# northflank-examples/distributed-pytorch-example

Measured on AMD Instinct MI355X. Metric: samples/sec (whole node) + DDP scaling eff., ResNet-50 bf16 at 1/2/4/8 MI355X, higher is better.
Workload: dtype bf16; 1 GPU; model=resnet50-v1.5, global_batch=512, per_gpu_batch=512, grad_accum=1, parallelism=dp1, optimizer=sgd-momentum0.9

## Files before the change

### csrc/bindings/bn.cpp

```cpp
#include <algorithm>
#include <vector>

#include "../kernels/pwconv.h"
#include "gemm_plan.h"
#include "ops_common.h"

namespace dpe_ops {
namespace {

int64_t rows_of(const Tensor& x) { return x.numel() / x.size(-1); }

std::vector<Tensor> bn_fwd_train(const Tensor& x, const c10::optional<Tensor>& gamma, const c10::optional<Tensor>& beta,
                                 const c10::optional<Tensor>& rmean, const c10::optional<Tensor>& rvar, double momentum,
                                 double eps, bool relu, const c10::optional<Tensor>& residual,
                                 const c10::optional<Tensor>& stats) {
  CHECK_GPU(x); CHECK_BF16(x); CHECK_CONTIG(x);
  const int64_t C = x.size(-1), M = rows_of(x);
  TORCH_CHECK(C % 8 == 0 && C <= 2048, "bn: C must be a multiple of 8 and <= 2048");
  auto fo = x.options().dtype(at::kFloat);
  Tensor coef = at::empty({4, C}, fo);
  hipStream_t st = cur_stream();
  if (has(stats)) {
    TORCH_CHECK(stats->dim() == 3 && stats->size(0) == 2 && stats->size(1) == C, "stats must be [2][C][nb] partials");
    CHECK_RC(dpe_bn_finalize(fp(*stats), (int)stats->size(2), (int)C, M, fpo(gamma), fpo(beta), fpom(rmean), fpom(rvar),
// ... 182 lines not shown
  const int64_t M = xshape[0] * xshape[1] * xshape[2], C = xshape[3];
  return (C == 64 || C == 128) && cmid == C && dpe_pw_cat_fwd_rowgroups(M, cout, C) > 0;
}

std::vector<Tensor> conv1x1_apply_cat(const Tensor& x, const Tensor& w, const c10::optional<Tensor>& in_coef,
                                      const Tensor& out_coef, const Tensor& x2, const Tensor& w2, const Tensor& coef2) {
  CHECK_GPU(x); CHECK_BF16(x); CHECK_CONTIG(x); CHECK_BF16(w); CHECK_CONTIG(w); CHECK_F32(out_coef); CHECK_CONTIG(out_coef);
  CHECK_GPU(x2); CHECK_BF16(x2); CHECK_CONTIG(x2); CHECK_BF16(w2); CHECK_CONTIG(w2); CHECK_F32(coef2); CHECK_CONTIG(coef2);
  const int64_t K1 = x.size(-1), M = x.numel() / K1, N = w.size(0), K2 = x2.size(-1);
  TORCH_CHECK(x.dim() == 4 && K1 == K2 && x2.numel() == M * K2 && w.numel() == N * K1 && w2.numel() == N * K2 &&
                  out_coef.numel() == 4 * N && coef2.numel() == 4 * N, "conv1x1_apply_cat: shapes");
  if (has(in_coef)) {
    CHECK_F32((*in_coef)); CHECK_CONTIG((*in_coef));
    TORCH_CHECK(in_coef->numel() == 4 * K1, "conv1x1_apply_cat: in_coef must be the BN's [4][K] coefficients");
  }
  TORCH_CHECK(down_cat_ok(x2.sizes().vec(), K1, N, 1), "conv1x1_apply_cat: outside the envelope (down_cat_ok)");
  const int rg = dpe_pw_cat_fwd_rowgroups(M, N, K2);
  auto ysz = x.sizes().vec();
  ysz.back() = N;
  Tensor y = at::empty(ysz, x.options());
  auto bsz = ysz;
  bsz.back() = N / 8;
  Tensor bits = at::empty(bsz, x.options().dtype(at::kByte));
  dpe::PwArgs pa{};
  pa.x = bp(x); pa.w = bp(w); pa.y = bpm(y);
  pa.x2 = bp(x2); pa.w2 = bp(w2); pa.cat_k2 = (int)K2;
  pa.in_coef = fpo(in_coef);
  pa.out_coef = fp(out_coef);
  pa.res_coef = fp(coef2);
  pa.out_bits = (uint8_t*)bits.data_ptr();
  pa.M = M; pa.N = N; pa.K = K1 + K2; pa.rg = rg; pa.sched = dpe_gemm::sched_buffer(cur_stream());
  CHECK_RC(dpe_pw_launch(&pa, dpe::PW_CAT, cur_stream()), "pw_stream concatenated-K apply");
  return {y, bits};
}

std::vector<Tensor> bn_gram_bwd(const Tensor& part, const Tensor& P, const Tensor& w, const Tensor& u, const Tensor& sv,
                                const Tensor& coef, const c10::optional<Tensor>& gamma, int64_t M,
                                const c10::optional<Tensor>& dgamma, const c10::optional<Tensor>& dbeta, Tensor& dw) {
  CHECK_GPU(part); CHECK_F32(part); CHECK_F32(P); CHECK_F32(u); CHECK_F32(sv); CHECK_F32(coef); CHECK_F32(dw);
  CHECK_BF16(w); CHECK_CONTIG(w); CHECK_CONTIG(P); CHECK_CONTIG(dw); CHECK_CONTIG(part);
  const int64_t Cout = w.size(0), Cin = w.numel() / Cout;
  TORCH_CHECK(part.dim() == 3 && part.size(1) == Cout && P.numel() == Cout * Cin && u.numel() == Cout * Cin &&
                  dw.numel() == Cout * Cin && sv.numel() == 2 * Cin && coef.numel() == 4 * Cout && sv.is_contiguous(),
              "bn_gram_bwd: shapes");
  auto fo = P.options();
  Tensor bcat = at::empty({Cout + Cin, Cin}, w.options()), abc = at::empty({3, Cout}, fo), e = at::empty({Cin}, fo);
  Tensor qws = at::empty({dpe_gram_bwd_ws_floats((int)Cin, (int)Cout)}, fo);
  CHECK_RC(dpe_gram_bwd(fp(part), (int)part.size(2), fp(P), bp(w), fp(u), fp(sv), fp(coef), fpo(gamma), (int)Cin,
                        (int)Cout, M, fpom(dgamma), fpom(dbeta), fp(dw), bpm(bcat), fp(abc), fp(e), fp(qws), cur_stream()),
           "bn_gram_bwd");
  return {bcat, e};
}

std::vector<Tensor> conv1x1_dgrad_cat(const Tensor& dz, const Tensor& a2src, const c10::optional<Tensor>& a2_coef,
                                      const Tensor& bcat, const Tensor& e, const Tensor& bn_x, const Tensor& bn_coef) {
  CHECK_GPU(dz); CHECK_BF16(dz); CHECK_CONTIG(dz); CHECK_BF16(a2src); CHECK_CONTIG(a2src); CHECK_BF16(bcat);
  CHECK_CONTIG(bcat); CHECK_F32(e); CHECK_BF16(bn_x); CHECK_CONTIG(bn_x); CHECK_F32(bn_coef);
  const int64_t K1 = dz.size(-1), M = dz.numel() / K1, C = a2src.size(-1);
  TORCH_CHECK(a2src.numel() == M * C && bcat.size(0) == K1 + C && bcat.size(1) == C && e.numel() == C &&
                  bn_x.sizes() == a2src.sizes() && bn_coef.numel() == 4 * C && K1 % 32 == 0 && C % 32 == 0,
              "conv1x1_dgrad_cat: shapes");
  Tensor dx = at::empty_like(bn_x);
  if (hgemm_conv_on() && !has(a2_coef) && C >= 256 && C % 64 == 0 && K1 % 64 == 0) {
    int pcols = 0;
    const auto pl = dpe_gemm::plan_bnb(M, C, K1 + C, 1, 0, &pcols);
    if (pl.cfg >= 0 && pl.splits == 1 && pcols > 0) {
// ... 364 lines not shown

}

void register_bn(pybind11::module& m) {
  namespace py = pybind11;
  m.def("gram_ok", [](std::vector<int64_t> h2shape, int64_t cout3, int64_t next_width) {
          if (h2shape.size() != 4 || !pw_stream_on()) return false;
          const int64_t M = h2shape[0] * h2shape[1] * h2shape[2], C2 = h2shape[3];
          if (C2 != 64 && C2 != 128 && C2 != 256) return false;
          if (cout3 % 128 || M % 32) return false;
          return dpe_pw_rowgroups(M, cout3, C2, dpe::PW_APPLY) > 0 &&
                 dpe_pw_rowgroups(M, cout3, next_width, dpe::PW_DSUM) > 0;
        }, py::arg("h2_shape"), py::arg("cout3"), py::arg("next_width"));
  m.def("bn_gram", &bn_gram, py::arg("x"), py::arg("coef") = py::none(), py::arg("shift_coef") = py::none(),
        py::arg("stride2") = false,
        "(G = a'^T a', s = [colsum(a'), mu]) of a' = a2 - mu, a2 = relu(x * coef[0] + coef[1]) (or x), centred on the "
        "pilot shift of shift_coef (default coef); fp32, deterministic");
  m.def("bn_gram_coef", &bn_gram_coef, py::arg("G"), py::arg("s"), py::arg("w"), py::arg("M"), py::arg("gamma"),
        py::arg("beta"), py::arg("running_mean"), py::arg("running_var"), py::arg("momentum"), py::arg("eps"),
        "BN coefficients [4][Cout] of the never-computed h = a2 W^T from (G, s), and u = W G");
  m.def("conv1x1_apply", &conv1x1_apply, py::arg("x"), py::arg("w"), py::arg("in_coef"), py::arg("out_coef"),
        py::arg("residual"), py::arg("res_coef") = py::none(),
        "y = relu(BN(x' W^T) + residual [BN_d]) and its ReLU bits (pre-BN tensor never stored)");
  m.def("conv1x1_apply_next", &conv1x1_apply_next, py::arg("x"), py::arg("w"), py::arg("in_coef"), py::arg("out_coef"),
        py::arg("residual"), py::arg("res_coef"), py::arg("w_next"), py::arg("outs") = py::none(),
        "conv1x1_apply's (y, bits) and, from the same pass, the next conv1's h1 = y W_next^T with its BN-forward partials");
  m.def("c1_fuse_ok", &c1_fuse_ok, py::arg("h2_shape"), py::arg("cout3"), py::arg("c1_next"),
        "conv1x1_apply_next's envelope: conv3 64 -> 256 beside a 1x1 stride-1 conv1 256 -> {64, 128}; no CU budget");
  m.def("conv1x1_apply_cat", &conv1x1_apply_cat, py::arg("x"), py::arg("w"), py::arg("in_coef"), py::arg("out_coef"),
        py::arg("x2"), py::arg("w2"), py::arg("coef2"),
        "y = relu(BN3(x' W^T) + BN_d(x2 W2^T)) over the concatenated K and its ReLU bits (no pre-BN tensors)");
  m.def("down_cat_ok", &down_cat_ok, py::arg("xshape"), py::arg("cmid"), py::arg("cout"), py::arg("stride"),
        "conv1x1_apply_cat's envelope: 1x1 stride-1 downsample conv, Cin == cmid in {64, 128}, cout == 4 Cin");
  m.def("bn_gram_bwd", &bn_gram_bwd, py::arg("part"), py::arg("P"), py::arg("w"), py::arg("u"), py::arg("s"),
        py::arg("coef"), py::arg("gamma"), py::arg("M"), py::arg("dgamma"), py::arg("dbeta"), py::arg("dw"),
        "BN3 backward from (sum dz partials, P = dz^T a2): dgamma/dbeta/dw +=, returns (B_cat bf16, bias)");
  m.def("conv1x1_dgrad_cat", &conv1x1_dgrad_cat, py::arg("dz"), py::arg("a2src"), py::arg("a2_coef"), py::arg("bcat"),
        py::arg("e"), py::arg("bn_x"), py::arg("bn_coef"),
        "[dz | a2] x bcat + e with the BN2-backward partials (concatenated-K data grad)");
  m.def("bn_gram_pilot", &bn_gram_pilot, py::arg("x"), py::arg("stride2") = false,
        "pilot shift [4][C] for bn_gram's shift_coef from a sample of x's rows (x without a producing BN)");
  m.def("bn_gram_u", &bn_gram_u, py::arg("G"), py::arg("w"), "u = W G (fp32) alone: no coefficients, no running stats");
  m.def("conv1x1_dgrad_cat_plain", &conv1x1_dgrad_cat_plain, py::arg("dz"), py::arg("x"), py::arg("bcat"), py::arg("e"),
        py::arg("stride2") = false,
        "[dz | x] x bcat + e (concatenated-K data grad of a Gram-path downsample branch, no partials)");
  m.def("bnd_gram_ok", [](std::vector<int64_t> xshape, int64_t cout, std::vector<int64_t> stride) {
          if (xshape.size() != 4 || stride.size() != 2 || stride[0] != stride[1] || !igemm_dma_on()) return false;
          const int64_t M = xshape[0] * xshape[1] * xshape[2], C = xshape[3];
          if (stride[0] == 1) return (C == 64 || C == 128) && cout == 4 * C && dpe_pw_cat_blocks(M, cout, C) > 0;
          if (stride[0] != 2 || xshape[1] % 2 || xshape[2] % 2) return false;
          static const bool gdma = env_on("DPE_GRAM_DMA", true);
          const int64_t Mo = M / 4, lim = (1ll << 31) - 4096;
          return gdma && (C == 64 || C == 128 || C == 256) && cout >= 256 && cout % 32 == 0 && hgemm_conv_on() &&
                 hgemm_conv_wgrad_on() && Mo % 64 == 0 && Mo < (1 << 24) && M * C * 2 < lim && Mo * cout * 2 < lim;
        }, py::arg("xshape"), py::arg("cout"), py::arg("stride"));
  m.def("bn_bwd_coef", &bn_bwd_coef, py::arg("partials"), py::arg("M"), py::arg("gamma"), py::arg("coef"),
        py::arg("dgamma") = py::none(), py::arg("dbeta") = py::none(),
        "BN-backward coefficients [3][C] from the dgrad-epilogue partials (no apply pass); dgamma/dbeta +=");
  m.def("conv1x1_bnin_fwd", &conv1x1_bnin_fwd, py::arg("h"), py::arg("res"), py::arg("coef"), py::arg("res_coef"),
        py::arg("w"), py::arg("x_out"), py::arg("x_bits"), py::arg("want_stats") = true, py::arg("tile_m") = 128,
        "1x1 conv over x = relu(BN(h) + res [BN_d]) computed on load; x (+ ReLU bits) stored as a by-product");
  m.def("conv1x1_bnin_dgrad", &conv1x1_bnin_dgrad, py::arg("dz"), py::arg("h"), py::arg("bcoef"), py::arg("w"),
        py::arg("dh_out"), py::arg("bn_x"), py::arg("bn_coef"),
        "1x1 data grad over dh = a*dz + b*h + c computed on load (dh stored as a by-product) + BN-backward partials");
  m.def("bn_coef", &bn_coef, py::arg("stats"), py::arg("M"), py::arg("gamma"), py::arg("beta"), py::arg("running_mean"),
        py::arg("running_var"), py::arg("momentum"), py::arg("eps"));
// ... 30 lines not shown
```

### csrc/kernels/pwconv.h

```cpp
#pragma once
#include <hip/hip_runtime.h>
#include <stdint.h>

namespace dpe {

enum PwEpi : int {
  PW_FWD = 0,
  PW_DGRAD = 1,
  PW_APPLY = 2,
  PW_DSUM = 3,
  PW_CAT = 4,
};

struct PwArgs {
  const uint16_t* x;
  const uint16_t* w;
  uint16_t* y;
  float* stats;
  const uint16_t* residual;
  const uint8_t* res_mask;
  const uint16_t* st_x;
  const float* st_coef;
  const uint8_t* st_mask;
  int64_t M, N, K;
// ... 11 lines not shown
  const uint16_t* x2;
  const uint16_t* w2;
  int cat_k2;
  const uint16_t* w_next;
  uint16_t* y_next;
  float* stats_next;
  int c1_next;
};

struct PwCatArgs {
  const uint16_t* dz;
  const uint16_t* h2;
  const float* coef;
  const uint16_t* bcat;
  const float* ebias;
  uint16_t* y;
  float* stats;
  int64_t M;
  int rg;
};

}

extern "C" int dpe_pw_cat_blocks(int64_t M, int64_t K1, int64_t K2);
extern "C" int dpe_pw_cat_launch(const dpe::PwCatArgs* args, int64_t K1, int64_t K2, hipStream_t stream);

extern "C" int dpe_pw_rowgroups(int64_t M, int64_t N, int64_t K, int epi);
extern "C" int dpe_pw_launch(const dpe::PwArgs* args, int epi, hipStream_t stream);

extern "C" int dpe_pw_cat_fwd_rowgroups(int64_t M, int64_t N, int64_t k2);

extern "C" int dpe_pw_p_rowgroups(int64_t M, int64_t N, int64_t K, int64_t k2);
extern "C" int dpe_pw_next_rowgroups(int64_t M, int64_t N, int64_t K, int64_t c1);

extern "C" int dpe_pw_p_reduce(const float* slab, int rg, int64_t n, float* P, hipStream_t stream);
```

### csrc/kernels/pwconv.hip

```cpp
#include <algorithm>
#include <cstdlib>

#include "common.h"
#include "igemm.h"
#include "launch.h"
#include "pwconv.h"

namespace dpe {
namespace pw {

constexpr int BM = 64;
typedef __attribute__((address_space(3))) void lds_void_t;

DPE_DEVICE int kimg_off(int row, int chunk) {
  const int g = (0x78 >> (((row >> 2) & 3) << 1)) & 3;
  return row * 64 + ((chunk ^ g) << 4);
}
DPE_DEVICE bf16x8 kfrag(const char* img, int r0) {
  const int lane = threadIdx.x & 63;
  return __builtin_bit_cast(bf16x8, *(const u32x4*)(img + kimg_off(r0 + (lane & 15), lane >> 4)));
}
DPE_DEVICE __amdgpu_buffer_rsrc_t rsrc(const void* base, uint32_t bytes) {
  return __builtin_amdgcn_make_buffer_rsrc(const_cast<void*>(base), (short)0, (int)bytes, 0x00020000);
}
template <int N>
DPE_DEVICE void wait_vm() {
  static_assert(N >= 0 && N < 64, "vmcnt");
  asm volatile("" ::: "memory");
  __builtin_amdgcn_s_waitcnt((N & 15) | (7 << 4) | (15 << 8) | ((N >> 4) << 14));
  asm volatile("" ::: "memory");
}

template <int C>
DPE_DEVICE int p_h(int row) {
  return C >= 128 ? ((row & 3) | (((row >> 3) & 1) << 2)) : (((row >> 1) & 1) | (((row >> 3) & 1) << 1));
}
typedef __attribute__((address_space(3))) s16x4 lds_s16x4_t;
DPE_DEVICE bf16x8 p_trfrag(const char* a1, const char* a2) {
  const s16x4 lo = __builtin_amdgcn_ds_read_tr16_b64_v4i16((lds_s16x4_t*)a1);
  const s16x4 hi = __builtin_amdgcn_ds_read_tr16_b64_v4i16((lds_s16x4_t*)a2);
  s16x8 r;
  r[0] = lo[0]; r[1] = lo[1]; r[2] = lo[2]; r[3] = lo[3];
  r[4] = hi[0]; r[5] = hi[1]; r[6] = hi[2]; r[7] = hi[3];
  return __builtin_bit_cast(bf16x8, r);
}

template <int K, int WN, int NS, int EPI, bool DYN = false, int K2 = 0, int C1 = 0>
__global__ __launch_bounds__(256, (K == 64 && (EPI == PW_FWD || (K2 > 0 && !DYN))) ? 3 : 2) void pw_stream_kernel(PwArgs a) {
  constexpr int KC = K / 32;
  constexpr int TILE = BM * K * 2;
  constexpr int P = TILE / 1024 / 4;
  constexpr int NI = WN / 16, MI = BM / 16;
  static_assert(P >= 1 && P * 4096 == TILE, "pieces");
  constexpr int ROWB = WN * 2 + 16, CPRW = WN / 8, RPP = 64 / CPRW, NPS = 32 / RPP;
  constexpr int STG = 32 * ROWB;
  constexpr bool NX = C1 > 0;
  static_assert(!NX || (EPI == PW_APPLY && K == 64 && WN == 64 && K2 == 0 && !DYN && (C1 == 64 || C1 == 128)), "next conv1: envelope");
  constexpr int HP = NX ? C1 / 64 : 0;
  constexpr int S = (EPI == PW_APPLY || EPI == PW_CAT ? 4 : 2) * NPS + 2 * HP;
  constexpr int VM = (NX && (NS - 1) * S + (NS - 2) * P > 63) ? 63 : (NS - 1) * S + (NS - 2) * P;
  static_assert(VM < 64, "vmcnt range");
  constexpr bool CAT = EPI == PW_CAT;
  static_assert(!CAT || (WN == 32 && 2 * K2 == K && K2 % 64 == 0), "concatenated K: envelope");
  constexpr int KS = CAT ? K2 : K;
  constexpr int KC1 = KS / 32;
  constexpr bool PF = K2 > 0 && !CAT;
  static_assert(!PF || (EPI == PW_DSUM && WN == 32 && (K2 == 64 || K2 == 128) && K2 <= K), "fused P: envelope");
  constexpr int A2OFF = NS * TILE + 4 * STG + 2 * K * 4 + 16, A2RB = 2 * (PF ? K2 : 8);
  constexpr int H1RB = C1 * 2 + 16, HCPR = NX ? C1 / 8 : 8, HRPP = 64 / HCPR;
  __shared__ __attribute__((aligned(16))) char smem[A2OFF + (PF ? BM * A2RB : NX ? 32 * H1RB : 0)];
  float* const bnin = (float*)(smem + NS * TILE + 4 * STG);
  int* const claim_slot = (int*)(smem + NS * TILE + 4 * STG + 2 * K * 4);

  constexpr bool DG = EPI == PW_DGRAD || EPI == PW_DSUM;
  const int tid = threadIdx.x, lane = tid & 63, g = lane >> 4, li = lane & 15;
  const int wid = __builtin_amdgcn_readfirstlane(tid >> 6);
  const int M = (int)a.M, N = (int)a.N, RG = a.rg;
  const int nbN = N / (4 * WN);
  const int bid = xcd_remap(blockIdx.x, gridDim.x);
  const int nb = bid % nbN;
  int rg = bid / nbN;
  const int SRG = (int)gridDim.x / nbN;
  const int n0w = nb * 4 * WN + wid * WN;
  const int tiles = (M + BM - 1) / BM;
  const int ch = lane % CPRW;
  const int nch = n0w + ch * 8;

  bf16x8 wf[NI][KC];
#pragma unroll
  for (int ni = 0; ni < NI; ++ni)
#pragma unroll
    for (int kc = 0; kc < KC; ++kc) {
      const int n = n0w + 16 * ni + li, k0 = 32 * kc + 8 * g;
      if constexpr (CAT) {
        const uint16_t* const ws = kc < KC1 ? a.w : a.w2;
        wf[ni][kc] = __builtin_bit_cast(bf16x8, *(const u32x4*)(ws + (int64_t)n * KS + (k0 - (kc < KC1 ? 0 : KS))));
      } else if constexpr (!DG) {
        wf[ni][kc] = __builtin_bit_cast(bf16x8, *(const u32x4*)(a.w + (int64_t)n * K + k0));
      } else {
        s16x8 v;
#pragma unroll
        for (int e = 0; e < 8; ++e) v[e] = (short)a.w[(int64_t)(k0 + e) * N + n];
        wf[ni][kc] = __builtin_bit_cast(bf16x8, v);
// ... 58 lines not shown
#pragma unroll
      for (int nj = 0; nj < PNJ; ++nj) pacc[ni][nj] = f32x4{0.f, 0.f, 0.f, 0.f};
  }
  float osc[8], osh[8], rsc[8], rsh[8];
  if constexpr (EPI == PW_APPLY) {
#pragma unroll
    for (int e = 0; e < 8; ++e) {
      osc[e] = a.out_coef[nch + e];
      osh[e] = a.out_coef[N + nch + e];
      rsc[e] = (!NX && a.res_coef) ? a.res_coef[nch + e] : 1.f;
      rsh[e] = (!NX && a.res_coef) ? a.res_coef[N + nch + e] : 0.f;
    }
  }
  const int rh = a.res_h, rw = a.res_w;
  auto res_off = [&](int m) -> int64_t {
    if (rh <= 0) return (int64_t)m * N + nch;
    const int hw = rh * rw, n = m / hw, r = m - n * hw, h = r / rw, w = r - h * rw;
    if ((h | w) & 1) return -1;
    return ((int64_t)(n * (rh >> 1) + (h >> 1)) * (rw >> 1) + (w >> 1)) * N + nch;
  };

  constexpr uint32_t OOB = 0xfffffff0u;
  const uint32_t ybytes = (uint32_t)((int64_t)M * N * 2), mbytes = (uint32_t)((int64_t)M * N / 8);
  const uint32_t rbytes = rh > 0 ? (uint32_t)((int64_t)(M / (rh * rw)) * (rh >> 1) * (rw >> 1) * N * 2) : ybytes;
  const __amdgpu_buffer_rsrc_t yrs = rsrc(a.y, ybytes);
  const __amdgpu_buffer_rsrc_t rrs = rsrc(a.residual, a.residual ? rbytes : 0u);
  const __amdgpu_buffer_rsrc_t rmrs = rsrc(a.res_mask, a.res_mask ? mbytes : 0u);
  const __amdgpu_buffer_rsrc_t xsrs = rsrc(a.st_x, bnx ? ybytes : 0u);
  const __amdgpu_buffer_rsrc_t smrs = rsrc(a.st_mask, (bnb && a.st_mask) ? mbytes : 0u);
  const __amdgpu_buffer_rsrc_t obrs = rsrc(a.out_bits, ((EPI == PW_APPLY || CAT) && a.out_bits) ? mbytes : 0u);
  const __amdgpu_buffer_rsrc_t psrs = rsrc(a.p_src, PF ? (uint32_t)((int64_t)M * K2 * 2) : 0u);
  const __amdgpu_buffer_rsrc_t h1rs = rsrc(a.y_next, NX ? (uint32_t)((int64_t)M * C1 * 2) : 0u);

  if (!DG && a.in_coef) {
    for (int i = tid; i < 2 * KS; i += 256) bnin[i] = a.in_coef[i];
    __syncthreads();
  }
  float c1s[CAT ? NI : 1][4], c2s[CAT ? NI : 1][4], cbs[CAT ? NI : 1][4];
  if constexpr (CAT) {
#pragma unroll
    for (int ni = 0; ni < NI; ++ni)
#pragma unroll
      for (int e = 0; e < 4; ++e) {
        const int n = n0w + 16 * ni + 4 * g + e;
        c1s[ni][e] = a.out_coef[n];
        c2s[ni][e] = a.res_coef[n];
        cbs[ni][e] = a.out_coef[N + n] + a.res_coef[N + n];
      }
  }
  if constexpr (PF) {
    if (a.p_coef)
      for (int i = tid; i < 2 * K2; i += 256) bnin[i] = a.p_coef[i];
    __syncthreads();
  }

  auto tile_body = [&](const int m0, const int cur_slot, const int nxt_tile, const int nxt_slot) {
    constexpr bool HOIST = (EPI != PW_FWD) && (WN == 32 || NX);
    constexpr bool HLD = HOIST && !CAT;
    constexpr int HN = HLD ? NPS : 1;
    u32x4 hrv[2][HN], hxv[2][HN];
    uint32_t hrmb[2][HN], hsmb[2][HN];
    if constexpr (HLD) {
#pragma unroll
      for (int hf = 0; hf < 2; ++hf)
#pragma unroll
        for (int ps = 0; ps < HN; ++ps) {
          const int m = min(m0 + 32 * hf + ps * RPP + lane / CPRW, M - 1);
          const int64_t off = (int64_t)m * N + nch;
          const int64_t ro = EPI == PW_APPLY ? off : res_off(m);
          if (a.residual) hrv[hf][ps] = __builtin_amdgcn_raw_buffer_load_b128(rrs, ro >= 0 ? (uint32_t)(ro * 2) : OOB, 0, 0);
          if constexpr (DG) {
            if (a.res_mask) hrmb[hf][ps] = __builtin_amdgcn_raw_buffer_load_b8(rmrs, (uint32_t)(off >> 3), 0, 0);
// ... 69 lines not shown
      wait_vm<P>();
      char* const a2 = smem + A2OFF;
      if (a.p_coef) {
        int ol = lane;
        asm volatile("" : "+v"(ol));
#pragma unroll
        for (int k = 0; k < PPW; ++k) {
          const int q = wid * PPW + k, r = q * PRPP + ol / PCPR, lc = (ol % PCPR) ^ (2 * p_h<K2>(r));
          const f32x4 s0 = *(const f32x4*)(bnin + 8 * lc), s1 = *(const f32x4*)(bnin + 8 * lc + 4);
          const f32x4 h0 = *(const f32x4*)(bnin + K2 + 8 * lc), h1 = *(const f32x4*)(bnin + K2 + 8 * lc + 4);
          const float sc8[8] = {s0[0], s0[1], s0[2], s0[3], s1[0], s1[1], s1[2], s1[3]};
          const float sh8[8] = {h0[0], h0[1], h0[2], h0[3], h1[0], h1[1], h1[2], h1[3]};
          u32x4* const pc = (u32x4*)(a2 + q * 1024 + ol * 16);
          float f[8];
          unpack8(*pc, f);
#pragma unroll
          for (int e = 0; e < 8; ++e) f[e] = fmaxf(fmaf(f[e], sc8[e], sh8[e]), 0.f);
          *pc = pack8(f);
        }
      }
    }
    char* stg = smem + NS * TILE + wid * STG;
#pragma unroll
    for (int hf = 0; hf < 2; ++hf) {
      if constexpr (NX) {
#pragma unroll
        for (int kc = 0; kc < KC; ++kc) {
          bf16x8 xf[2];
#pragma unroll
          for (int mh = 0; mh < 2; ++mh) xf[mh] = kfrag(img + kc * (BM * 64), 16 * (2 * hf + mh));
#pragma unroll
          for (int mh = 0; mh < 2; ++mh)
#pragma unroll
            for (int ni = 0; ni < NI; ++ni)
              acc[2 * hf + mh][ni] = __builtin_amdgcn_mfma_f32_16x16x32_bf16(wf[ni][kc], xf[mh], acc[2 * hf + mh][ni], 0, 0, 0);
        }
      }
      u32x4 rv[NPS], xv[NPS];
      uint32_t rmb[NPS], smb[NPS];
      if constexpr (HLD) {
#pragma unroll
        for (int ps = 0; ps < HN; ++ps) {
          rv[ps] = hrv[hf][ps];
          xv[ps] = hxv[hf][ps];
          rmb[ps] = a.res_mask ? hrmb[hf][ps] : 0xffu;
          smb[ps] = (bnb && a.st_mask) ? hsmb[hf][ps] : 0xffu;
        }
      } else if constexpr (DG) {
#pragma unroll
        for (int ps = 0; ps < NPS; ++ps) {
          const int m = min(m0 + 32 * hf + ps * RPP + lane / CPRW, M - 1);
          const int64_t off = (int64_t)m * N + nch;
          if (a.residual) {
            const int64_t ro = res_off(m);
            rv[ps] = ro >= 0 ? *(const u32x4*)(a.residual + ro) : u32x4{0u, 0u, 0u, 0u};
          }
          rmb[ps] = a.res_mask ? (uint32_t)a.res_mask[off >> 3] : 0xffu;
          if (bnx) xv[ps] = *(const u32x4*)(a.st_x + off);
          smb[ps] = (bnb && a.st_mask) ? (uint32_t)a.st_mask[off >> 3] : 0xffu;
        }
      }
#pragma unroll
      for (int mh = 0; mh < 2; ++mh) {
        const int mi = 2 * hf + mh;
#pragma unroll
        for (int ni = 0; ni < NI; ++ni) {
          if constexpr (CAT) {
#pragma unroll
            for (int e = 0; e < 4; ++e)
              acc[mi][ni][e] = fmaxf(fmaf(acc[mi][ni][e], c1s[ni][e], fmaf(acc2[mi][ni][e], c2s[ni][e], cbs[ni][e])), 0.f);
          }
          u32x2 pk;
          pk[0] = pack_bf2(acc[mi][ni][0], acc[mi][ni][1]);
          pk[1] = pack_bf2(acc[mi][ni][2], acc[mi][ni][3]);
          *(u32x2*)(stg + (16 * mh + li) * ROWB + (16 * ni + 4 * g) * 2) = pk;
        }
      }
      if (HLD && hf == 0) wait_vm<P>();
#pragma unroll
      for (int ps = 0; ps < NPS; ++ps) {
        const int row = ps * RPP + lane / CPRW;
        u32x4 v = *(const u32x4*)(stg + row * ROWB + ch * 16);
        const int m = m0 + 32 * hf + row;
        const bool valid = m < M;
        float f[8];
        unpack8(v, f);
        if constexpr (EPI == PW_APPLY) {
          float r[8];
          if (a.residual) unpack8(rv[ps], r);
#pragma unroll
          for (int e = 0; e < 8; ++e) {
            float t = fmaf(f[e], osc[e], osh[e]);
            if (a.residual) t += (!NX && a.res_coef) ? bf2f(f2bf(fmaf(r[e], rsc[e], rsh[e]))) : r[e];
            f[e] = fmaxf(t, 0.f);
          }
          v = pack8(f);
          if constexpr (HOIST)
            __builtin_amdgcn_raw_buffer_store_b8(relu_mask_byte(v), obrs, valid ? (uint32_t)(((int64_t)m * N + nch) >> 3) : OOB, 0, 0);
          else if (valid && a.out_bits)
            a.out_bits[((int64_t)m * N + nch) >> 3] = relu_mask_byte(v);
// ... 523 lines not shown
  }
  if (K != 64 && K != 128 && K != 256) return {0, 0};
  if (epi != PW_FWD && epi != PW_DGRAD && epi != PW_APPLY && epi != PW_DSUM && epi != PW_CAT) return {0, 0};
  const int bnb = 4 * pw_wn((int)K, epi);
  if (N % bnb || N < 2 * K) return {0, 0};
  if (M * K * 2 >= (1ll << 31) - 4096 || M * N >= (1ll << 31) - 256) return {0, 0};
  const int64_t tiles = (M + pw::BM - 1) / pw::BM;
  const int64_t nbN = N / bnb;
  const int reserve = dpe_cu_reserve();
  if (reserve > 0 && pw_dynamic()) {
    if (k2 == 128 && epi != PW_CAT) return {0, 0};
    const int64_t srg = std::max<int64_t>(1, (pw_cap<true>(K, epi, k2) - reserve) / nbN);
    static const int64_t fac = [] { const char* e = getenv("DPE_PW_DYN_FACTOR"); return (int64_t)(e ? std::max(2, atoi(e)) : 8); }();
    const int64_t rg = std::min<int64_t>(fac * srg, tiles / 7);
    if (rg > srg) return {(int)rg, (int)srg};
  }
  int64_t rg = (pw_cap<false>(K, epi, k2) - reserve) / nbN;
  rg = std::max<int64_t>(1, std::min<int64_t>(rg, tiles));
  return {(int)rg, (int)rg};
}

static int pw_plan_next(int64_t M, int64_t N, int64_t K, int64_t c1) {
  if (K != 64 || N != 256 || (c1 != 64 && c1 != 128)) return 0;
  if (M <= 0 || M * N >= (1ll << 31) - 256) return 0;
  const int reserve = dpe_cu_reserve();
  if (reserve > 0 && pw_dynamic()) return 0;
  const int cap = c1 == 64 ? pw_slots<64, 64, 4, PW_APPLY, false, 0, 64>() : pw_slots<64, 64, 4, PW_APPLY, false, 0, 128>();
  const int64_t tiles = (M + pw::BM - 1) / pw::BM;
  return (int)std::max<int64_t>(1, std::min<int64_t>(cap - reserve, tiles));
}

extern "C" int dpe_pw_next_rowgroups(int64_t M, int64_t N, int64_t K, int64_t c1) { return pw_plan_next(M, N, K, c1); }

extern "C" int dpe_pw_rowgroups(int64_t M, int64_t N, int64_t K, int epi) { return pw_plan(M, N, K, epi).rg; }

extern "C" int dpe_pw_cat_fwd_rowgroups(int64_t M, int64_t N, int64_t k2) {
  return (k2 > 0 && N == 4 * k2) ? pw_plan(M, N, 2 * k2, PW_CAT, k2).rg : 0;
}

extern "C" int dpe_pw_p_rowgroups(int64_t M, int64_t N, int64_t K, int64_t k2) {
  return k2 > 0 ? pw_plan(M, N, K, PW_DSUM, k2).rg : 0;
}

__global__ __launch_bounds__(256) void pw_p_reduce_kernel(const float* __restrict__ slab, int rg, int64_t n,
                                                          float* __restrict__ P) {
  __shared__ float part[8][32];
  const int o = threadIdx.x & 31, q = threadIdx.x >> 5;
  const int64_t i = (int64_t)blockIdx.x * 32 + o;
  float t = 0.f;
  if (i < n) {
    int r = q;
    for (; r + 56 < rg; r += 64) {
      float v[8];
#pragma unroll
      for (int k = 0; k < 8; ++k) v[k] = slab[(int64_t)(r + 8 * k) * n + i];
#pragma unroll
      for (int k = 0; k < 8; ++k) t += v[k];
    }
    for (; r < rg; r += 8) t += slab[(int64_t)r * n + i];
  }
  part[q][o] = t;
  __syncthreads();
  if (q == 0 && i < n) {
    float u = 0.f;
#pragma unroll
    for (int k = 0; k < 8; ++k) u += part[k][o];
    P[i] = u;
  }
}

extern "C" int dpe_pw_p_reduce(const float* slab, int rg, int64_t n, float* P, hipStream_t st) {
  if (rg <= 0 || n <= 0) return -1;
  hipLaunchKernelGGL(pw_p_reduce_kernel, dim3((unsigned)((n + 31) / 32)), dim3(256), 0, st, slab, rg, n, P);
  return 0;
}

extern "C" int dpe_pw_launch(const PwArgs* args, int epi, hipStream_t st) {
  const PwArgs& a = *args;
  if (a.p_k2 < 0 || (a.p_k2 > 0 && (epi != PW_DSUM || !a.p_src || !a.p_slab))) return -1;
  if ((epi == PW_CAT) != (a.cat_k2 > 0) || (epi == PW_CAT && a.p_k2 > 0)) return -1;
  if (a.c1_next != 0) {
    if (epi != PW_APPLY || a.p_k2 != 0 || !a.w_next || !a.y_next || !a.stats_next || !a.out_coef || !a.residual || a.res_coef ||
        !a.out_bits || a.st_x || a.stats || a.res_h > 0)
      return -1;
    if (a.rg <= 0 || a.rg != pw_plan_next(a.M, a.N, a.K, a.c1_next)) return -1;
    const dim3 grid((unsigned)a.rg), block(256);
    if (a.c1_next == 64) hipLaunchKernelGGL((pw::pw_stream_kernel<64, 64, 4, PW_APPLY, false, 0, 64>), grid, block, 0, st, a);
    else hipLaunchKernelGGL((pw::pw_stream_kernel<64, 64, 4, PW_APPLY, false, 0, 128>), grid, block, 0, st, a);
    return 0;
  }
  const int64_t k2 = epi == PW_CAT ? a.cat_k2 : a.p_k2;
  if (a.rg <= 0 || a.rg != pw_plan(a.M, a.N, a.K, epi, k2).rg) return -1;
  if (epi == PW_CAT && (!a.x2 || !a.w2 || !a.out_coef || !a.res_coef || !a.out_bits || a.residual || a.st_x || a.stats ||
                        a.res_h > 0))
    return -1;
  if (epi == PW_FWD && (a.residual || a.st_x)) return -1;
  if (a.st_x && !a.st_coef) return -1;
  if (epi == PW_DSUM && (a.st_x || !a.st_mask || !a.stats)) return -1;
  if (epi == PW_APPLY && (!a.out_coef || a.st_x || a.stats || a.res_h > 0 || (a.res_coef && !a.residual))) return -1;
  if (a.res_h > 0 && ((epi != PW_DGRAD && epi != PW_DSUM) || a.res_mask || a.res_h % 2 || a.res_w % 2 || a.M % ((int64_t)a.res_h * a.res_w)))
    return -1;
  const int srg = a.sched ? pw_plan(a.M, a.N, a.K, epi, k2).srg : a.rg;
  const bool dyn = srg < a.rg;
  const int wn = pw_wn((int)a.K, epi);
  const dim3 grid((unsigned)(srg * (a.N / (4 * wn)))), block(256);
#define PW_GO(K_, WN_, NS_, E_)                                                                            \
  if (a.K == K_ && wn == WN_ && epi == E_) {                                                             \
    if (dyn) hipLaunchKernelGGL((pw::pw_stream_kernel<K_, WN_, NS_, E_, true>), grid, block, 0, st, a);    \
    else hipLaunchKernelGGL((pw::pw_stream_kernel<K_, WN_, NS_, E_, false>), grid, block, 0, st, a);       \
    return 0;                                                                                            \
  }
#define PW_GO_P(K_, NS_, K2_)                                                                                \
  if (a.K == K_ && a.p_k2 == K2_) {                                                                        \
// ... 32 lines not shown
```

### distributed_pytorch_example_amd/models/_resnet_fused.py

```python
from __future__ import annotations

import os

import torch
from torch.autograd import Function

from ..ops._ext import ext
from ..ops._state import finalize_stream, grad_done, grad_sink, note_use, run_on_aux, shadow

_EPI_BNB = os.environ.get("DPE_BN_EPI", "1") != "0"
_BN3_CHAIN = _EPI_BNB and os.environ.get("DPE_BN3_CHAIN", "1") != "0"
_BN_DUAL = os.environ.get("DPE_BN_DUAL", "1") != "0"
_ROW_BNIN = _EPI_BNB and os.environ.get("DPE_ROW_BNIN", "1") != "0"
_PW_BNIN = _EPI_BNB and os.environ.get("DPE_PW_BNIN", "1") != "0"
_DOWN_CHAIN = _BN3_CHAIN and os.environ.get("DPE_DOWN_CHAIN", "1") != "0"
_AX_FWD = _BN3_CHAIN and os.environ.get("DPE_AX_FWD", "0") == "1"
_AX_BWD = _BN3_CHAIN and os.environ.get("DPE_AX_BWD", "0") == "1"
_AX_BWD_MAXC = int(os.environ.get("DPE_AX_BWD_MAXC", "512"))
_AX_TILE = int(os.environ.get("DPE_AX_TILE", "256"))
_GRAM = _BN3_CHAIN and os.environ.get("DPE_BN3_GRAM", "1") != "0"
_BND_GRAM = _GRAM and os.environ.get("DPE_BND_GRAM", "1") != "0"
_BND_GRAM_S2 = _BND_GRAM and os.environ.get("DPE_BND_GRAM_S2", "0") == "1"
_PW_FUSED_P = _GRAM and os.environ.get("DPE_PW_FUSED_P", "1") != "0"
_DOWN_CAT =_BND_GRAM and os.environ.get("DPE_DOWN_CAT", "1") != "0"
_C1_FUSE = _GRAM and os.environ.get("DPE_C1_FUSE", "1") != "0"


def _ax_ok(conv, cin) -> bool:
    return (tuple(conv.kernel_size) == (1, 1) and tuple(conv.stride) == (1, 1) and tuple(conv.padding) == (0, 0)
            and cin % 32 == 0 and cin <= 2048)


def can_materialise_input(block) -> bool:
    return _AX_FWD and block.fused and _ax_ok(block.c1.conv, block.c1.conv.in_channels)


def _out_hw(hw, conv):
    k, s, p, d = conv.kernel_size[0], conv.stride[0], conv.padding[0], conv.dilation[0]
    return (hw + 2 * p - d * (k - 1) - 1) // s + 1


class _BN3Link:

    __slots__ = ("h3", "coef", "mask", "part", "dz_ptr", "dz_shape", "pending", "gram", "psrc", "P", "h1_next")

    def __init__(self):
        self.h3 = self.coef = self.mask = self.part = None
        self.psrc = self.P = None
        self.dz_ptr, self.dz_shape = 0, None
        self.gram = False
        self.pending = None
        self.h1_next = None


def _conv_conf(conv):
    return list(conv.stride), list(conv.padding), list(conv.dilation)


# ... 34 lines not shown
        def conv_coef(i, inp, in_coef=None):
            cb = convs[i]
            s, p, d = _conv_conf(cb.conv)
            if i == 0 and h1_done is not None:
                h, st = h1_done
            else:
                h, st = C.conv_fwd(inp, ws[i], s, p, d, True, None, in_coef)
            bn = cb.bn
            M = h.numel() // h.shape[-1]
            return h, C.bn_coef(st, M, bn.weight.detach(), bn.bias.detach(), bn.running_mean, bn.running_var, bn.momentum,
                                bn.eps)

        c1conv, c2conv = convs[0].conv, convs[1].conv
        h1_shape = [x.shape[0], _out_hw(x.shape[1], c1conv), _out_hw(x.shape[2], c1conv), c1conv.out_channels]
        h2_shape = [x.shape[0], _out_hw(h1_shape[1], c2conv), _out_hw(h1_shape[2], c2conv), c2conv.out_channels]
        out_shape = [*h2_shape[:3], convs[2].conv.out_channels]
        dconv = block.down.conv if block.down is not None else None
        use_gram = bool(gram_next and link_out is not None and not defer_out and h1_st is None
                        and (gram_next > 0 or C.pw_dgrad_strided_residual_ok(out_shape, -gram_next))
                        and C.gram_ok(h2_shape, convs[2].conv.out_channels, abs(gram_next)))
        bnd_gram = bool(use_gram and _BND_GRAM and dconv is not None and tuple(dconv.kernel_size) == (1, 1)
                        and tuple(dconv.padding) == (0, 0)
                        and C.bnd_gram_ok(list(x.shape), dconv.out_channels, list(dconv.stride))
                        and (tuple(dconv.stride) == (1, 1) or (_BND_GRAM_S2 and tuple(c1conv.stride) == (1, 1) and
                             C.pw_dgrad_strided_residual_ok(list(x.shape), c1conv.out_channels))))
        down_cat = bool(use_gram and _DOWN_CAT and dconv is not None and tuple(dconv.kernel_size) == (1, 1)
                        and tuple(dconv.padding) == (0, 0) and tuple(dconv.stride) == (1, 1)
                        and C.down_cat_ok(list(x.shape), h2_shape[3], dconv.out_channels, 1))
        c1n = next_block.c1.conv if next_block is not None else None
        c1_fuse = bool(use_gram and _C1_FUSE and c1n is not None and block.down is None and gram_next
                       and tuple(c1n.kernel_size) == (1, 1) and tuple(c1n.stride) == (1, 1)
                       and tuple(c1n.padding) == (0, 0) and c1n.in_channels == out_shape[3] and c1n.out_channels == abs(gram_next)
                       and C.c1_fuse_ok(h2_shape, out_shape[3], c1n.out_channels))
        if h1_st is None and block.down is not None and not down_cat:
            hd, cd = conv_coef(3, x)
        else:
            hd, cd = None, None
        if _ROW_BNIN and C.row_bn_on_load(h1_shape, list(ws[1].shape), *_conv_conf(c2conv)):
            h1, c1 = conv_coef(0, x)
            a1 = None
            h2, st2 = C.conv_fwd(h1, ws[1], *_conv_conf(c2conv), True, None, c1)
        else:
            h1, a1, c1 = convbn(0, x, True)
            h2, st2 = C.conv_fwd(a1, ws[1], *_conv_conf(c2conv), True, None)
        if h1_st is not None and block.down is not None:
            hd, cd = conv_coef(3, x)
        bn2 = convs[1].bn
        if _PW_BNIN and C.pw_bn_on_load(list(h2.shape), convs[2].conv.out_channels):
            c2 = C.bn_coef(st2, h2.numel() // h2.shape[-1], bn2.weight.detach(), bn2.bias.detach(),
                           bn2.running_mean, bn2.running_var, bn2.momentum, bn2.eps)
            a2 = None
        else:
            a2, c2 = C.bn_fwd_train(h2, bn2.weight.detach(), bn2.bias.detach(), bn2.running_mean,
                                    bn2.running_var, bn2.momentum, bn2.eps, True, None, st2)
        want_bits = True
        gram = None
        bnd = None
        assert list(h2.shape) == h2_shape
        if use_gram:
            src, src_coef = (h2, c2) if a2 is None else (a2, None)
            G, sv = C.bn_gram(src, src_coef, c2)
            bn3 = convs[2].bn
            M3 = h2.numel() // h2.shape[-1]
            c3, u3 = C.bn_gram_coef(G, sv, ws[2], M3, bn3.weight.detach(), bn3.bias.detach(), bn3.running_mean,
                                    bn3.running_var, bn3.momentum, bn3.eps)
            if down_cat:
                bnd_ = convs[3].bn
                Gx, sx = C.bn_gram(x, None, C.bn_gram_pilot(x, False), False)
                cd, ud = C.bn_gram_coef(Gx, sx, ws[3], M3, bnd_.weight.detach(), bnd_.bias.detach(), bnd_.running_mean,
                                        bnd_.running_var, bnd_.momentum, bnd_.eps)
                out, bits = C.conv1x1_apply_cat(src, ws[2], src_coef, c3, x, ws[3], cd)
                if bnd_gram:
                    bnd = (ud, sx)
                else:
                    hd = C.conv_fwd(x, ws[3], *_conv_conf(dconv), False, None)[0]
            elif block.down is not None:
                out, bits = C.conv1x1_apply(src, ws[2], src_coef, c3, hd, cd)
            elif c1_fuse:
                out, bits, nh1, nst = C.conv1x1_apply_next(src, ws[2], src_coef, c3, x, None, shadow(c1n.weight))
                link_out.h1_next = (nh1, nst, out, next_block)
            else:
                out, bits = C.conv1x1_apply(src, ws[2], src_coef, c3, x, None)
            h3 = None
            gram = (u3, sv, M3)
            if bnd_gram and not down_cat:
                s2 = tuple(dconv.stride) == (2, 2)
                Gx, sx = C.bn_gram(x, None, C.bn_gram_pilot(x, s2), s2)
                bnd = (C.bn_gram_u(Gx, ws[3]), sx)
        else:
            h3, c3 = conv_coef(2, h2, c2) if a2 is None else conv_coef(2, a2)
        if gram is not None:
            pass
        elif defer_out and link_out is not None:
            out = torch.empty_like(h3)
            bits = torch.empty(*h3.shape[:-1], h3.shape[-1] // 8, dtype=torch.uint8, device=h3.device)
            link_out.pending = (h3, c3, hd, cd, out, bits) if block.down is not None else (h3, c3, x, None, out, bits)
        elif block.down is not None:
            out, bits = C.bn_apply(h3, c3, hd, cd, True, want_bits)
        else:
            out, bits = C.bn_apply(h3, c3, x, None, True, want_bits)
        ctx.save_for_backward(x, h1, a1, h2, a2, h3, out, None if bnd is not None else hd, c1, c2, c3, cd)
        strided_ok = block.down is not None and _DOWN_CHAIN and tuple(block.down.conv.stride) == (2, 2) and \
            tuple(block.down.conv.kernel_size) == (1, 1) and tuple(convs[0].conv.stride) == (1, 1) and \
            C.pw_dgrad_strided_residual_ok(list(x.shape), convs[0].conv.out_channels)
# ... 285 lines not shown
```

Measured before the change: 17660 samples/s.

## Fuse next block's conv1 into the concatenated-K downsample apply kernel

Adds a PW_CAT variant of the pointwise streaming kernel that, while writing the first bottleneck block's output (conv3 plus downsample over concatenated K), also computes the next block's conv1 h1 = y W_next^T and its BN-forward partials. This targets layer1's first block (64->256 with a stride-1 downsample) and avoids re-reading y from memory for a separate conv1 and stats pass. In exchange the CAT path now splits MFMA accumulation into acc and acc2 by K half and keeps a shared-memory coefficient table, which costs extra registers and LDS and may reduce occupancy.

```diff
diff --git a/csrc/bindings/bn.cpp b/csrc/bindings/bn.cpp
--- a/csrc/bindings/bn.cpp
+++ b/csrc/bindings/bn.cpp
@@ -238,6 +238,62 @@
   pa.M = M; pa.N = N; pa.K = K1 + K2; pa.rg = rg; pa.sched = dpe_gemm::sched_buffer(cur_stream());
   CHECK_RC(dpe_pw_launch(&pa, dpe::PW_CAT, cur_stream()), "pw_stream concatenated-K apply");
   return {y, bits};
+}
+
+bool c1_fuse_cat_ok(const std::vector<int64_t>& xshape, int64_t cmid, int64_t cout, int64_t c1_next) {
+  if (!down_cat_ok(xshape, cmid, cout, 1) || !pw_stream_on()) return false;
+  const int64_t M = xshape[0] * xshape[1] * xshape[2];
+  return cmid == 64 && cout == 256 && c1_next == 64 && dpe_pw_cat_next_rowgroups(M, cout, cmid, c1_next) > 0;
+}
+
+std::vector<Tensor> conv1x1_apply_cat_next(const Tensor& x, const Tensor& w, const c10::optional<Tensor>& in_coef,
+                                           const Tensor& out_coef, const Tensor& x2, const Tensor& w2, const Tensor& coef2,
+                                           const Tensor& w_next, const c10::optional<std::vector<Tensor>>& outs) {
+  CHECK_GPU(x); CHECK_BF16(x); CHECK_CONTIG(x); CHECK_GPU(w); CHECK_BF16(w); CHECK_CONTIG(w);
+  CHECK_GPU(out_coef); CHECK_F32(out_coef); CHECK_CONTIG(out_coef);
+  CHECK_GPU(x2); CHECK_BF16(x2); CHECK_CONTIG(x2); CHECK_GPU(w2); CHECK_BF16(w2); CHECK_CONTIG(w2);
+  CHECK_GPU(coef2); CHECK_F32(coef2); CHECK_CONTIG(coef2); CHECK_GPU(w_next); CHECK_BF16(w_next); CHECK_CONTIG(w_next);
+  TORCH_CHECK(x.dim() == 4 && x2.dim() == 4, "conv1x1_apply_cat_next: x and x2 must be [N, H, W, K]");
+  const int64_t K1 = x.size(-1), M = x.numel() / K1, N = w.size(0), K2 = x2.size(-1), C1 = w_next.size(0);
+  TORCH_CHECK(K1 == K2 && x2.numel() == M * K2 && w.numel() == N * K1 && w2.numel() == N * K2 && out_coef.numel() == 4 * N &&
+                  coef2.numel() == 4 * N && w_next.numel() == C1 * N, "conv1x1_apply_cat_next: shapes");
+  if (has(in_coef)) {
+    CHECK_GPU((*in_coef)); CHECK_F32((*in_coef)); CHECK_CONTIG((*in_coef));
+    TORCH_CHECK(in_coef->numel() == 4 * K1, "conv1x1_apply_cat_next: in_coef must be the BN's [4][K] coefficients");
+  }
+  TORCH_CHECK(c1_fuse_cat_ok(x2.sizes().vec(), K1, N, C1), "conv1x1_apply_cat_next: outside the envelope (c1_fuse_cat_ok)");
+  const int rg = dpe_pw_cat_next_rowgroups(M, N, K2, C1);
+  auto ysz = x.sizes().vec();
+  ysz.back() = N;
+  Tensor y = at::empty(ysz, x.options());
+  auto bsz = ysz;
+  bsz.back() = N / 8;
+  Tensor bits = at::empty(bsz, x.options().dtype(at::kByte));
+  auto hsz = ysz;
+  hsz.back() = C1;
+  Tensor h1 = at::empty(hsz, x.options());
+  Tensor st = at::empty({2, C1, rg}, x.options().dtype(at::kFloat));
+  if (outs.has_value()) {
+    TORCH_CHECK(outs->size() == 4, "conv1x1_apply_cat_next: outs must be (y, bits, h1, st)");
+    const Tensor* mine[4] = {&y, &bits, &h1, &st};
+    for (int i = 0; i < 4; ++i) {
+      const Tensor& o = (*outs)[i];
+      TORCH_CHECK(o.is_cuda() && o.is_contiguous() && o.sizes() == mine[i]->sizes() && o.scalar_type() == mine[i]->scalar_type(),
+                  "conv1x1_apply_cat_next: outs[", i, "] has the wrong shape, type or layout");
+    }
+    y = (*outs)[0]; bits = (*outs)[1]; h1 = (*outs)[2]; st = (*outs)[3];
+  }
+  dpe::PwArgs pa{};
+  pa.x = bp(x); pa.w = bp(w); pa.y = bpm(y);
+  pa.x2 = bp(x2); pa.w2 = bp(w2); pa.cat_k2 = (int)K2;
+  pa.in_coef = fpo(in_coef);
+  pa.out_coef = fp(out_coef);
+  pa.res_coef = fp(coef2);
+  pa.out_bits = (uint8_t*)bits.data_ptr();
+  pa.w_next = bp(w_next); pa.y_next = bpm(h1); pa.stats_next = fp(st); pa.c1_next = (int)C1;
+  pa.M = M; pa.N = N; pa.K = K1 + K2; pa.rg = rg;
+  CHECK_RC(dpe_pw_launch(&pa, dpe::PW_CAT, cur_stream()), "pw_stream concatenated-K apply + next conv1");
+  return {y, bits, h1, st};
 }
 
 std::vector<Tensor> bn_gram_bwd(const Tensor& part, const Tensor& P, const Tensor& w, const Tensor& u, const Tensor& sv,
@@ -668,6 +724,11 @@
         "y = relu(BN3(x' W^T) + BN_d(x2 W2^T)) over the concatenated K and its ReLU bits (no pre-BN tensors)");
   m.def("down_cat_ok", &down_cat_ok, py::arg("xshape"), py::arg("cmid"), py::arg("cout"), py::arg("stride"),
         "conv1x1_apply_cat's envelope: 1x1 stride-1 downsample conv, Cin == cmid in {64, 128}, cout == 4 Cin");
+  m.def("conv1x1_apply_cat_next", &conv1x1_apply_cat_next, py::arg("x"), py::arg("w"), py::arg("in_coef"), py::arg("out_coef"),
+        py::arg("x2"), py::arg("w2"), py::arg("coef2"), py::arg("w_next"), py::arg("outs") = py::none(),
+        "conv1x1_apply_cat's (y, bits) and, from the same pass, the next conv1's h1 = y W_next^T with its BN-forward partials");
+  m.def("c1_fuse_cat_ok", &c1_fuse_cat_ok, py::arg("xshape"), py::arg("cmid"), py::arg("cout"), py::arg("c1_next"),
+        "conv1x1_apply_cat_next's envelope: down_cat_ok at 64 -> 256 beside a 1x1 stride-1 conv1 256 -> 64; no CU budget");
   m.def("bn_gram_bwd", &bn_gram_bwd, py::arg("part"), py::arg("P"), py::arg("w"), py::arg("u"), py::arg("s"),
         py::arg("coef"), py::arg("gamma"), py::arg("M"), py::arg("dgamma"), py::arg("dbeta"), py::arg("dw"),
         "BN3 backward from (sum dz partials, P = dz^T a2): dgamma/dbeta/dw +=, returns (B_cat bf16, bias)");
diff --git a/csrc/kernels/pwconv.h b/csrc/kernels/pwconv.h
--- a/csrc/kernels/pwconv.h
+++ b/csrc/kernels/pwconv.h
@@ -67,5 +67,6 @@
 
 extern "C" int dpe_pw_p_rowgroups(int64_t M, int64_t N, int64_t K, int64_t k2);
 extern "C" int dpe_pw_next_rowgroups(int64_t M, int64_t N, int64_t K, int64_t c1);
+extern "C" int dpe_pw_cat_next_rowgroups(int64_t M, int64_t N, int64_t k2, int64_t c1);
 
 extern "C" int dpe_pw_p_reduce(const float* slab, int rg, int64_t n, float* P, hipStream_t stream);
diff --git a/csrc/kernels/pwconv.hip b/csrc/kernels/pwconv.hip
--- a/csrc/kernels/pwconv.hip
+++ b/csrc/kernels/pwconv.hip
@@ -55,20 +55,25 @@
   constexpr int ROWB = WN * 2 + 16, CPRW = WN / 8, RPP = 64 / CPRW, NPS = 32 / RPP;
   constexpr int STG = 32 * ROWB;
   constexpr bool NX = C1 > 0;
-  static_assert(!NX || (EPI == PW_APPLY && K == 64 && WN == 64 && K2 == 0 && !DYN && (C1 == 64 || C1 == 128)), "next conv1: envelope");
+  static_assert(!NX || (WN == 64 && !DYN && ((EPI == PW_APPLY && K == 64 && K2 == 0 && (C1 == 64 || C1 == 128)) ||
+                                             (EPI == PW_CAT && K == 128 && K2 == 64 && C1 == 64))),
+                "next conv1: envelope");
   constexpr int HP = NX ? C1 / 64 : 0;
   constexpr int S = (EPI == PW_APPLY || EPI == PW_CAT ? 4 : 2) * NPS + 2 * HP;
   constexpr int VM = (NX && (NS - 1) * S + (NS - 2) * P > 63) ? 63 : (NS - 1) * S + (NS - 2) * P;
   static_assert(VM < 64, "vmcnt range");
   constexpr bool CAT = EPI == PW_CAT;
-  static_assert(!CAT || (WN == 32 && 2 * K2 == K && K2 % 64 == 0), "concatenated K: envelope");
+  static_assert(!CAT || ((WN == 32 || NX) && 2 * K2 == K && K2 % 64 == 0), "concatenated K: envelope");
+  constexpr bool CN = CAT && NX;
+  constexpr int CTN = 4 * WN;
   constexpr int KS = CAT ? K2 : K;
   constexpr int KC1 = KS / 32;
   constexpr bool PF = K2 > 0 && !CAT;
   static_assert(!PF || (EPI == PW_DSUM && WN == 32 && (K2 == 64 || K2 == 128) && K2 <= K), "fused P: envelope");
   constexpr int A2OFF = NS * TILE + 4 * STG + 2 * K * 4 + 16, A2RB = 2 * (PF ? K2 : 8);
   constexpr int H1RB = C1 * 2 + 16, HCPR = NX ? C1 / 8 : 8, HRPP = 64 / HCPR;
-  __shared__ __attribute__((aligned(16))) char smem[A2OFF + (PF ? BM * A2RB : NX ? 32 * H1RB : 0)];
+  constexpr int CTOFF = A2OFF + 32 * H1RB;
+  __shared__ __attribute__((aligned(16))) char smem[A2OFF + (PF ? BM * A2RB : NX ? 32 * H1RB : 0) + (CN ? 3 * CTN * 4 : 0)];
   float* const bnin = (float*)(smem + NS * TILE + 4 * STG);
   int* const claim_slot = (int*)(smem + NS * TILE + 4 * STG + 2 * K * 4);
 
@@ -193,12 +198,22 @@
   const __amdgpu_buffer_rsrc_t psrs = rsrc(a.p_src, PF ? (uint32_t)((int64_t)M * K2 * 2) : 0u);
   const __amdgpu_buffer_rsrc_t h1rs = rsrc(a.y_next, NX ? (uint32_t)((int64_t)M * C1 * 2) : 0u);
 
+  if constexpr (CN) {
+    float* const ctab = (float*)(smem + CTOFF);
+    for (int n = tid; n < CTN; n += 256) {
+      ctab[n] = a.out_coef[n];
+      ctab[CTN + n] = a.res_coef[n];
+      ctab[2 * CTN + n] = a.out_coef[N + n] + a.res_coef[N + n];
+    }
+  }
   if (!DG && a.in_coef) {
     for (int i = tid; i < 2 * KS; i += 256) bnin[i] = a.in_coef[i];
     __syncthreads();
-  }
-  float c1s[CAT ? NI : 1][4], c2s[CAT ? NI : 1][4], cbs[CAT ? NI : 1][4];
-  if constexpr (CAT) {
+  } else if constexpr (CN) {
+    __syncthreads();
+  }
+  float c1s[CAT && !CN ? NI : 1][4], c2s[CAT && !CN ? NI : 1][4], cbs[CAT && !CN ? NI : 1][4];
+  if constexpr (CAT && !CN) {
 #pragma unroll
     for (int ni = 0; ni < NI; ++ni)
 #pragma unroll
@@ -334,8 +349,15 @@
 #pragma unroll
           for (int mh = 0; mh < 2; ++mh)
 #pragma unroll
-            for (int ni = 0; ni < NI; ++ni)
+            for (int ni = 0; ni < NI; ++ni) {
+              if constexpr (CAT) {
+                if (kc >= KC1) {
+                  acc2[2 * hf + mh][ni] = __builtin_amdgcn_mfma_f32_16x16x32_bf16(wf[ni][kc], xf[mh], acc2[2 * hf + mh][ni], 0, 0, 0);
+                  continue;
+                }
+              }
               acc[2 * hf + mh][ni] = __builtin_amdgcn_mfma_f32_16x16x32_bf16(wf[ni][kc], xf[mh], acc[2 * hf + mh][ni], 0, 0, 0);
+            }
         }
       }
       u32x4 rv[NPS], xv[NPS];
@@ -367,7 +389,13 @@
         const int mi = 2 * hf + mh;
 #pragma unroll
         for (int ni = 0; ni < NI; ++ni) {
-          if constexpr (CAT) {
+          if constexpr (CN) {
+            const float* const ct = (const float*)(smem + CTOFF) + n0w + 16 * ni + 4 * g;
+            const f32x4 t1 = *(const f32x4*)ct, t2 = *(const f32x4*)(ct + CTN), tb = *(const f32x4*)(ct + 2 * CTN);
+#pragma unroll
+            for (int e = 0; e < 4; ++e)
+              acc[mi][ni][e] = fmaxf(fmaf(acc[mi][ni][e], t1[e], fmaf(acc2[mi][ni][e], t2[e], tb[e])), 0.f);
+          } else if constexpr (CAT) {
 #pragma unroll
             for (int e = 0; e < 4; ++e)
               acc[mi][ni][e] = fmaxf(fmaf(acc[mi][ni][e], c1s[ni][e], fmaf(acc2[mi][ni][e], c2s[ni][e], cbs[ni][e])), 0.f);
@@ -957,6 +985,18 @@
 
 extern "C" int dpe_pw_next_rowgroups(int64_t M, int64_t N, int64_t K, int64_t c1) { return pw_plan_next(M, N, K, c1); }
 
+static int pw_plan_cat_next(int64_t M, int64_t N, int64_t k2, int64_t c1) {
+  if (N != 256 || k2 != 64 || c1 != 64) return 0;
+  if (M <= 0 || M * N >= (1ll << 31) - 256) return 0;
+  const int reserve = dpe_cu_reserve();
+  if (reserve > 0 && pw_dynamic()) return 0;
+  const int cap = pw_slots<128, 64, 3, PW_CAT, false, 64, 64>();
+  const int64_t tiles = (M + pw::BM - 1) / pw::BM;
+  return (int)std::max<int64_t>(1, std::min<int64_t>(cap - reserve, tiles));
+}
+
+extern "C" int dpe_pw_cat_next_rowgroups(int64_t M, int64_t N, int64_t k2, int64_t c1) { return pw_plan_cat_next(M, N, k2, c1); }
+
 extern "C" int dpe_pw_rowgroups(int64_t M, int64_t N, int64_t K, int epi) { return pw_plan(M, N, K, epi).rg; }
 
 extern "C" int dpe_pw_cat_fwd_rowgroups(int64_t M, int64_t N, int64_t k2) {
@@ -1004,6 +1044,15 @@
   const PwArgs& a = *args;
   if (a.p_k2 < 0 || (a.p_k2 > 0 && (epi != PW_DSUM || !a.p_src || !a.p_slab))) return -1;
   if ((epi == PW_CAT) != (a.cat_k2 > 0) || (epi == PW_CAT && a.p_k2 > 0)) return -1;
+  if (a.c1_next != 0 && epi == PW_CAT) {
+    if (a.p_k2 != 0 || !a.x || !a.w || !a.y || !a.x2 || !a.w2 || !a.out_coef || !a.res_coef || !a.out_bits || !a.w_next ||
+        !a.y_next || !a.stats_next || a.residual || a.res_mask || a.st_x || a.st_mask || a.stats || a.res_h > 0 || a.sched)
+      return -1;
+    if (a.K != 2 * (int64_t)a.cat_k2) return -1;
+    if (a.rg <= 0 || a.rg != pw_plan_cat_next(a.M, a.N, a.cat_k2, a.c1_next)) return -1;
+    hipLaunchKernelGGL((pw::pw_stream_kernel<128, 64, 3, PW_CAT, false, 64, 64>), dim3((unsigned)a.rg), dim3(256), 0, st, a);
+    return 0;
+  }
   if (a.c1_next != 0) {
     if (epi != PW_APPLY || a.p_k2 != 0 || !a.w_next || !a.y_next || !a.stats_next || !a.out_coef || !a.residual || a.res_coef ||
         !a.out_bits || a.st_x || a.stats || a.res_h > 0)
diff --git a/distributed_pytorch_example_amd/models/_resnet_fused.py b/distributed_pytorch_example_amd/models/_resnet_fused.py
--- a/distributed_pytorch_example_amd/models/_resnet_fused.py
+++ b/distributed_pytorch_example_amd/models/_resnet_fused.py
@@ -24,6 +24,7 @@
 _PW_FUSED_P = _GRAM and os.environ.get("DPE_PW_FUSED_P", "1") != "0"
 _DOWN_CAT =_BND_GRAM and os.environ.get("DPE_DOWN_CAT", "1") != "0"
 _C1_FUSE = _GRAM and os.environ.get("DPE_C1_FUSE", "1") != "0"
+_C1_FUSE_CAT = _C1_FUSE and os.environ.get("DPE_C1_FUSE_CAT", "1") != "0"
 
 
 def _ax_ok(conv, cin) -> bool:
@@ -124,6 +125,11 @@
                        and tuple(c1n.kernel_size) == (1, 1) and tuple(c1n.stride) == (1, 1)
                        and tuple(c1n.padding) == (0, 0) and c1n.in_channels == out_shape[3] and c1n.out_channels == abs(gram_next)
                        and C.c1_fuse_ok(h2_shape, out_shape[3], c1n.out_channels))
+        c1_fuse_cat = bool(down_cat and _C1_FUSE_CAT and c1n is not None and gram_next
+                           and tuple(c1n.kernel_size) == (1, 1) and tuple(c1n.stride) == (1, 1)
+                           and tuple(c1n.padding) == (0, 0) and c1n.in_channels == out_shape[3]
+                           and c1n.out_channels == abs(gram_next)
+                           and C.c1_fuse_cat_ok(list(x.shape), h2_shape[3], dconv.out_channels, c1n.out_channels))
         if h1_st is None and block.down is not None and not down_cat:
             hd, cd = conv_coef(3, x)
         else:
@@ -161,7 +167,11 @@
                 Gx, sx = C.bn_gram(x, None, C.bn_gram_pilot(x, False), False)
                 cd, ud = C.bn_gram_coef(Gx, sx, ws[3], M3, bnd_.weight.detach(), bnd_.bias.detach(), bnd_.running_mean,
                                         bnd_.running_var, bnd_.momentum, bnd_.eps)
-                out, bits = C.conv1x1_apply_cat(src, ws[2], src_coef, c3, x, ws[3], cd)
+                if c1_fuse_cat:
+                    out, bits, nh1, nst = C.conv1x1_apply_cat_next(src, ws[2], src_coef, c3, x, ws[3], cd, shadow(c1n.weight))
+                    link_out.h1_next = (nh1, nst, out, next_block)
+                else:
+                    out, bits = C.conv1x1_apply_cat(src, ws[2], src_coef, c3, x, ws[3], cd)
                 if bnd_gram:
                     bnd = (ud, sx)
                 else:
```

Result: no change. 17740 samples/s (median of 6 runs) (+0.5%).
